# vladiant/CascadeClassifier

Measured on AMD Instinct MI355X. Metric: detection Mwindows/sec (1080p, haarcascade_frontalface) + achieved HBM GB/s, higher is better.
Workload: dtype i32+f32 (f64 stage sums)

## Files before the change

### cascadeclassifier_amd/_lib.py

```python
from __future__ import annotations

import ctypes as C
import os

_HERE = os.path.dirname(os.path.abspath(__file__))
LIB_PATH = os.environ.get("CCAMD_LIB") or os.path.join(_HERE, "lib", "libcascadeclassifier_amd.so")

CC_OK = 0
CC_ERR_INVALID_ARG = -1
CC_ERR_NO_DEVICE = -2
CC_ERR_HIP = -3
CC_ERR_IO = -4
CC_ERR_PARSE = -5
CC_ERR_UNSUPPORTED = -6
CC_ERR_BUFFER_TOO_SMALL = -7
CC_ERR_OUT_OF_RANGE = -8

CC_FEATURE_HAAR, CC_FEATURE_LBP, CC_FEATURE_HOG = 0, 1, 2
CC_PIX_GRAY8, CC_PIX_BGR8, CC_PIX_BGRA8, CC_PIX_RGB8, CC_PIX_RGBA8, CC_PIX_RGB8_PLANAR = 0, 1, 2, 3, 4, 5
CC_HAAR_BASIC, CC_HAAR_CORE, CC_HAAR_ALL = 0, 1, 2


class CascadeError(RuntimeError):

# ... 124 lines not shown
    "cc_detector_specialize": (_i, [_vp, _i]),
    "cc_detector_specialize_async": (_i, [_vp, _i]),
    "cc_detector_specialized_stages": (_i, [_vp]),
    "cc_cascade_compile_specialized": (_i, [_vp, _i, C.c_char_p, C.POINTER(C.c_size_t)]),
    "cc_detector_set_profiling": (_i, [_vp, _i]),
    "cc_detector_graph_active": (_i, [_vp]),
    "cc_detector_graph_captures": (C.c_int64, [_vp]),
    "cc_detector_get_timings": (_i, [_vp, C.POINTER(DetectorTimings), _i]),
    "cc_detector_candidate_capacity": (_i, [_vp]),
    "cc_integral_u8": (_i, [_i, _vp, _i, _i, _sz, _vp, _vp, _vp]),
    "cc_resize_linear_exact_u8": (_i, [_i, _vp, _i, _i, _sz, _vp, _i, _i, _sz]),
    "cc_debug_stream_dwords": (_i, [_i, _sz, _i, C.POINTER(C.c_uint32)]),
    "cc_debug_division_check": (_i, [_i, C.c_uint64, C.c_uint64, C.POINTER(C.c_uint64)]),
    "cc_debug_vnf_check": (_i, [_i, C.c_uint64, C.c_uint64, C.POINTER(C.c_uint64)]),
    "cc_debug_wave_int_tables": (_i, [_vp, _vp, _vp, _vp, _vp]),
    "cc_group_rectangles": (_i, [_vp, _i, _i, _d, _vp, _i, C.POINTER(_i)]),
    "cc_group_rectangles_device": (_i, [_i, _vp, _vp, _i, _i, _d, _vp, _i, _vp, C.POINTER(_i)]),
    "cc_group_rectangles_levels": (_i, [_vp, _vp, _vp, _i, _i, _d, _vp, _vp, _vp, _i, C.POINTER(_i)]),
    "cc_group_rectangles_device_levels": (_i, [_i, _vp, _vp, _vp, _vp, _i, _i, _d, _vp, _vp, _vp, _i, _vp, C.POINTER(_i)]),
    "cc_eval_create": (_i, [_i, _i, _i, _i, _i, _i, _pp]),
    "cc_eval_destroy": (None, [_vp]),
    "cc_eval_num_features": (_i, [_vp]),
    "cc_eval_max_cat_count": (_i, [_vp]),
    "cc_eval_feature_size": (_i, [_vp]),
    "cc_eval_feature_geometry": (_i, [_vp, _i, _vp, _vp, C.POINTER(_i)]),
    "cc_eval_set_image": (_i, [_vp, _vp, _sz, C.c_uint8, _i]),
    "cc_eval_set_images": (_i, [_vp, _vp, _i, _i, _vp]),
    "cc_eval_labels": (C.POINTER(C.c_float), [_vp]),
    "cc_eval_calc": (_i, [_vp, _i, _i, C.POINTER(C.c_float)]),
    "cc_eval_calc_list": (_i, [_vp, _vp, _i, _i, _vp]),
# ... 99 lines not shown
```

### cascadeclassifier_amd/csrc/cc_detect.hip

```cpp
#include <hip/hip_runtime.h>

#include <algorithm>

#include "cc_detector.h"

namespace ccamd {

#include "cc_eval_kernel.inc"

__global__ __launch_bounds__(256) void k_stream_dwords(const uint32_t* __restrict__ p, size_t n_words, uint32_t* __restrict__ out) {
  uint32_t acc = 0;
  for (size_t i = (size_t)blockIdx.x * blockDim.x + threadIdx.x; i < n_words; i += (size_t)gridDim.x * blockDim.x) acc += p[i];
  if (acc == 0x9e3779b9u) atomicAdd(out, acc);
  atomicAdd(out + 1 + (threadIdx.x & 15), acc);
}

__device__ __forceinline__ bool visited_by_scan(const unsigned long long* __restrict__ row_mask, int gx) {
  int run = 0;
  int pos = gx - 1;
  while (pos >= 0) {
    const int b = pos & 63;
    const unsigned long long w = row_mask[pos >> 6] << (63 - b);
    const int ones = min(__clzll((long long)~w), b + 1);
    run += ones;
// ... 115 lines not shown
  A.leaves = d->d_leaves.p;
  return A;
}

int eval_stamp_slots() { return STAMP_SLOTS; }

cc_status launch_eval(cc_detector* d, const Plan* P, int slot, int nchan, bool tilt, int sq_compact, bool debug, unsigned long long* stamps,
                      const EvalLaunch* launches, int n_launches, int nf, hipStream_t st) {
  const bool haar = d->m.feature_type == CC_FEATURE_HAAR;
  EvalArgs A = eval_args(d, P, slot, nchan, tilt, sq_compact, debug);
  A.stamps = stamps;
  for (int i = 0; i < n_launches; i++) {
    const EvalLaunch& L = launches[i];
    if (L.n_tiles == 0) continue;
    A.tiles = L.tiles;
    if (L.fn) {
      void* params[] = {&A};
      EvScope ev1(d, i == 1 ? EV_EVAL_STEP1 : -1, st);
      CC_HIP(hipModuleLaunchKernel(L.fn, (unsigned)L.n_tiles, (unsigned)nf, 1, EVAL_THREADS, 1, 1, (unsigned)L.lds, st, params, nullptr));
    } else if (haar)
      hipLaunchKernelGGL(k_eval_haar, dim3(L.n_tiles, nf), dim3(EVAL_THREADS), L.lds, st, A);
    else
      hipLaunchKernelGGL(k_eval_lbp, dim3(L.n_tiles, nf), dim3(EVAL_THREADS), L.lds, st, A);
    if (A.stamps) A.stamps += (size_t)L.n_tiles * (size_t)nf * STAMP_SLOTS;
  }
  return CC_OK;
}

void launch_filter_candidates(cc_detector* d, const Plan* P, int slot, hipStream_t st) {
  hipLaunchKernelGGL(k_filter_candidates, dim3(64), dim3(256), 0, st, d->d_cands[slot].p, d->d_counts[slot].p, d->cand_cap, P->front.d_sd.p,
// ... 64 lines not shown
```

### cascadeclassifier_amd/csrc/cc_detect_api.hip

```cpp
#include <algorithm>
#include <chrono>
#include <cstdlib>
#include <mutex>
#include <unordered_set>

#include "cc_detector.h"

namespace ccamd {

cc_status refuse_hog(const Cascade& m, const char* who) {
  if (m.feature_type == CC_FEATURE_HAAR || m.feature_type == CC_FEATURE_LBP) return CC_OK;
  return set_error(CC_ERR_UNSUPPORTED, "%s: %s cascades are not supported for detection (Haar and LBP only)", who,
                   m.feature_type == CC_FEATURE_HOG ? "HOG" : "unknown-type");
}

cc_status ensure_device(int device) {
  int n = 0;
  hipError_t e = hipGetDeviceCount(&n);
  if (e != hipSuccess || n <= 0)
    return set_error(CC_ERR_NO_DEVICE, "no usable HIP device (%s); this library has no CPU fallback",
                     e != hipSuccess ? hipGetErrorString(e) : "device count is 0");
  if (device < 0 || device >= n) return set_error(CC_ERR_INVALID_ARG, "device %d out of range (devices: %d)", device, n);
  CC_HIP(hipSetDevice(device));
  return CC_OK;
// ... 61 lines not shown
  sink->consume = [&cands](int, int, std::vector<CandOut>& c) { cands.insert(cands.end(), c.begin(), c.end()); };
  BatchOptions opt;
  opt.debug = debug;
  const cc_status st = run_batch(d, F, p, sink, opt);
  if (st == CC_OK) sort_candidates(cands);
  return st;
}

static cc_status spec_install(cc_detector* d, const std::vector<SpecCode>& codes, int k, int tmode) {
  retire_foreign(d);
  CC_HIP(hipStreamSynchronize(d->stream));
  SpecModule fresh[2];
  int n_fresh = 0;
  if (cc_status st = spec_load(d->m, codes, tmode, d->lds, fresh, &n_fresh); st != CC_OK) return st;
  d->unload_spec();
  for (int i = 0; i < n_fresh; i++) d->spec[i] = fresh[i];
  d->n_spec = n_fresh;
  d->spec_stages = k;
  return CC_OK;
}

static cc_status device_arch(int device, std::string& arch) {
  hipDeviceProp_t prop;
  CC_HIP(hipGetDeviceProperties(&prop, device));
  arch = prop.gcnArchName;
  arch = arch.substr(0, arch.find(':'));
  return CC_OK;
}

void spec_poll(cc_detector* d) {
  const int st = d->spec_bg_state.load(std::memory_order_acquire);
// ... 495 lines not shown
```

### cascadeclassifier_amd/csrc/cc_detect_internal.h

```cpp
#pragma once
#include <hip/hip_runtime.h>

#include <cstring>
#include <string>
#include <vector>

#include "cc_hip_util.h"
#include "cc_internal.h"

namespace ccamd {

#include "cc_eval_common.h"

__device__ __forceinline__ int find_segment(const int* __restrict__ first, int n, int idx) {
  int s = 0;
  while (s + 1 < n && first[s + 1] <= idx) s++;
  return s;
}

inline int align_up(int v, int a) { return (v + a - 1) / a * a; }

struct FrontLayout {
  int src_w = 0, src_h = 0;
  std::vector<ScaleDev> sd;
// ... 131 lines not shown

struct SpecCode {
  std::vector<char> code;
  int only_step = 0;
  int tile_y = TILE_Y;
};

cc_status spec_build(const Cascade& m, int n_stages, const std::string& arch, std::vector<SpecCode>& codes, int& k_out, int& tmode_out);

struct SpecModule {
  hipModule_t mod = nullptr;
  hipFunction_t fn = nullptr;
  size_t lds = 0;
  int tile_y = TILE_Y;
  int only_step = 0;
};

cc_status spec_load(const Cascade& m, const std::vector<SpecCode>& codes, int tmode, size_t base_lds, SpecModule out[2], int* n_out);

struct GroupGuard {
  const int* counts = nullptr;
  int cand_cap = 0;
  int* abort = nullptr;
};
constexpr int GROUP_WS_INTS = 7;
constexpr int GROUP_WS_INTS_SCORED = 10;
struct GroupScores {
  bool scored = false;
  const int32_t* levels = nullptr;
  int const_level = 0;
  const double* weights = nullptr;
// ... 18 lines not shown
```

### cascadeclassifier_amd/csrc/cc_detector.h

```cpp
#pragma once
#include <atomic>
#include <functional>
#include <future>
#include <map>
#include <memory>
#include <thread>

#include "cc_detect_internal.h"

namespace ccamd {

struct Plan {
  int w = 0, h = 0;
  cc_detect_params p{};
  std::vector<ScaleGeom> geom;
  FrontTables front;
  size_t mask_frame_words = 0;
  long long windows = 0, integral_elems = 0;
  int n_grid_rows = 0;
  struct TileList {
    int n = 0;
    DevBuf<int4> d;
  };
  std::map<std::pair<int, int>, TileList> tiles;
// ... 170 lines not shown
struct EvScope {
  cc_detector* d;
  int kind;
  OwnEvent a, b;
  hipStream_t st;
  EvScope(cc_detector* d_, int kind_, hipStream_t st_);
  ~EvScope();
};
void collect_events(cc_detector* d);

struct EvalLaunch {
  hipFunction_t fn;
  size_t lds;
  int n_tiles;
  const int4* tiles;
};
cc_status launch_eval(cc_detector* d, const Plan* P, int slot, int nchan, bool tilt, int sq_compact, bool debug, unsigned long long* stamps,
                      const EvalLaunch* launches, int n_launches, int nf, hipStream_t st);
int eval_stamp_slots();
void launch_filter_candidates(cc_detector* d, const Plan* P, int slot, hipStream_t st);
void launch_debug_visited(cc_detector* d, const Plan* P, int slot, hipStream_t st);
cc_status allow_large_lds(const cc_detector* d);

void configure_detector(cc_detector* d);
cc_status upload_cascade_tables(cc_detector* d);

cc_status build_plan(cc_detector* d, int w, int h, const cc_detect_params& p, Plan** out);
cc_status check_frame_args(const cc_detector* d, const FrameSet& F, const cc_detect_params* p, const char* who);
cc_status retire_pending(cc_detector* d);
void retire_foreign(cc_detector* d);
// ... 7 lines not shown
```

### cascadeclassifier_amd/csrc/cc_eval_common.h

```cpp
#ifndef CC_EVAL_COMMON_H
#define CC_EVAL_COMMON_H

constexpr int TILE_X = 64;
#ifndef CC_TILE_Y
#define CC_TILE_Y 8
#endif
#ifndef CC_EVAL_THREADS
#define CC_EVAL_THREADS 256
#endif
#ifndef CC_EVAL_MIN_WAVES_PER_EU
#define CC_EVAL_MIN_WAVES_PER_EU 5
#endif
constexpr int TILE_Y = CC_TILE_Y;
constexpr int EVAL_THREADS = CC_EVAL_THREADS;
constexpr int EVAL_WAVES = EVAL_THREADS / 64;
constexpr int WIN_PER_THREAD = TILE_Y / EVAL_WAVES;
constexpr int SPEC_PARTS = EVAL_WAVES >= 8 ? 8 : EVAL_WAVES >= 4 ? 4 : EVAL_WAVES >= 2 ? 2 : 1;

struct ScaleDev {
  int w, h;
  int pitch8, pitchI;
  long long img_ofs, int_ofs, mask_ofs, win_ofs, h_ofs;
  int ystep, nx, ny, nxw, nbands;
  float scale;
// ... 67 lines not shown
    rows = (tile_y - 1) * 2 + H0 + 1;
    rs16 = (cols + 3) / 4 * 4;
    if (rs16 % 16 == 0) rs16 += 4;
    row_stride = rs16 / 2;
  }
  __host__ __device__ int at(int r, int c) const { return r * rs16 + c; }
  __host__ __device__ int words() const { return rows * row_stride; }
};

constexpr int TILE_WINDOWS = TILE_X * TILE_Y;
constexpr int MAX_STAGES = 64;
constexpr int PART_DOUBLES = (EVAL_WAVES - 1) * 64;
constexpr int QUEUE_ROWS = TILE_WINDOWS / 32;
constexpr int VNF_PITCH = TILE_X + 32;
__host__ __device__ inline int tile_words_padded(int tile_words) { return (tile_words + 3) & ~3; }
__host__ __device__ inline size_t eval_lds_bytes(int tile_words, bool tilted, bool haar = true, int tile_y = TILE_Y) {
  return (size_t)tile_words_padded(tile_words) * 4 * (tilted ? 2 : 1) + PART_DOUBLES * 8 + (haar ? tile_y * VNF_PITCH * 4 : 0) +
         2 * (tile_y * TILE_X) * 2 + 3 * 32 * 4;
}

template <int CTRL, int ROW_MASK>
__device__ __forceinline__ double dpp_f64(double v) {
  const unsigned long long u = __double_as_longlong(v);
  const int lo = __builtin_amdgcn_update_dpp(0, (int)(unsigned)u, CTRL, ROW_MASK, 0xF, false);
  const int hi = __builtin_amdgcn_update_dpp(0, (int)(unsigned)(u >> 32), CTRL, ROW_MASK, 0xF, false);
  return __longlong_as_double(((unsigned long long)(unsigned)hi << 32) | (unsigned)lo);
}
__device__ __forceinline__ double readlane_f64(double v, int src) {
  const unsigned long long u = __double_as_longlong(v);
  const unsigned lo = __builtin_amdgcn_readlane((int)(unsigned)u, src);
  const unsigned hi = __builtin_amdgcn_readlane((int)(unsigned)(u >> 32), src);
  return __longlong_as_double(((unsigned long long)hi << 32) | lo);
}
// ... 15 lines not shown
```

### cascadeclassifier_amd/csrc/cc_eval_kernel.inc

```

#define CC_CONST __attribute__((address_space(4)))
template <class T>
__device__ __forceinline__ const T CC_CONST* as_const_table(const T* p) {
  return (const T CC_CONST*)p;
}
template <class T>
__device__ __forceinline__ T load_record(const T CC_CONST* p) {
  static_assert(sizeof(T) % 4 == 0, "table records are dword multiples");
  T out;
  const int CC_CONST* w = (const int CC_CONST*)p;
  int* o = reinterpret_cast<int*>(&out);
#pragma unroll
  for (unsigned i = 0; i < sizeof(T) / 4; i++) o[i] = w[i];
  return out;
}

constexpr int STAGE_ROWS = 12;
template <int STEP, class Geom>
__device__ __forceinline__ void stage_tile(int32_t* lds, const Geom& G, const int32_t* __restrict__ sum,
                                           const ScaleDev& S, int x0, int y0) {
  const int lane = threadIdx.x & 63, wave = __builtin_amdgcn_readfirstlane(threadIdx.x >> 6);
  const int quads = (G.cols + 3) >> 2;
  const bool right_edge = x0 + quads * 4 - 1 > S.w;
  for (int q0 = 0; q0 < quads; q0 += 64) {
// ... 262 lines not shown
#else
  static constexpr bool G16 = false;
#endif
  using Geom = typename cc_select<G16, TileGeom16, TileGeom<STEP>>::type;

  const EvalArgs& A;
  int32_t* const lds;
  const int4 T;
  const ScaleDev& S;
#ifdef CC_SPEC_W0
  static constexpr int W0 = CC_SPEC_W0, H0 = CC_SPEC_H0;
#else
  const int W0 = A.W0, H0 = A.H0;
#endif
  const Geom G{W0, H0};
  double* const s_part = reinterpret_cast<double*>(lds + tile_words_padded(G.words()) * ((HAAR && A.tilt_chan >= 0) ? 2 : 1));
  float* const s_vnf = reinterpret_cast<float*>(s_part + PART_DOUBLES);
  unsigned short* const s_q = reinterpret_cast<unsigned short*>(s_vnf + (HAAR ? TILE_Y * VNF_PITCH : 0));
  int* const s_cnt = reinterpret_cast<int*>(s_q + 2 * TILE_WINDOWS);
  const int frame = blockIdx.y;
  const int32_t* const sum = A.integ + ((size_t)frame * A.nchan + 0) * A.int_frame_elems + S.int_ofs;
  const int lane = threadIdx.x & 63, wave = __builtin_amdgcn_readfirstlane(threadIdx.x >> 6);
  const int half = lane >> 5, cls = lane & 31;
  const int gx0 = T.y * TILE_X, gy0 = T.z * TILE_Y;
  const int skew = (STEP * G.row_stride) & 31;
  const Node* const nodes = reinterpret_cast<const Node*>(STEP == 2 ? A.nodes2 : A.nodes1);
  const Stump CC_CONST* const stumps = as_const_table(reinterpret_cast<const Stump*>(G16 ? A.gstumps : STEP == 2 ? A.stumps2 : A.stumps1));
  const int CC_CONST* const stage_first = as_const_table(A.stage_first);
  const int CC_CONST* const stage_ntrees = as_const_table(A.stage_ntrees);
  const float CC_CONST* const stage_thr = as_const_table(A.stage_thr);
  const int CC_CONST* const group_first = as_const_table(A.group_first);
  const double CC_CONST* const wave_q = as_const_table(A.wave_q);
  const int CC_CONST* const wave_thr_q = as_const_table(A.wave_thr_q);
// ... 10 lines not shown
    if constexpr (G16)
      return GlobalReader{sum, (unsigned)((gy0 + (id >> 6)) * STEP) * (unsigned)S.pitchI + (unsigned)((gx0 + (id & 63)) * STEP), S.pitchI};
    else
      return LdsReader{lds + window_base(id)};
  }
  __device__ __forceinline__ void report(int id, int code, double last) const {
    const size_t o = (size_t)S.win_ofs + (size_t)(gy0 + (id >> 6)) * S.nx + (gx0 + (id & 63));
    A.dbg_codes[o] = code;
    if (A.dbg_sums) A.dbg_sums[o] = last;
  }
  __device__ __forceinline__ void emit_candidate(int id, double last_sum) const {
    const int slot = atomicAdd(A.cand_count, 1);
    if (slot < A.cand_cap) A.cands[slot] = CandRaw{frame, T.x, gx0 + (id & 63), gy0 + (id >> 6), last_sum};
  }
  __device__ __forceinline__ int win_class(int id) const { return ((id & 63) + skew * (id >> 6)) & 31; }
  __device__ __forceinline__ int vnf_slot(int id) const { return (id >> 6) * (TILE_X + skew) + (id & 63); }
  __device__ __forceinline__ void enqueue(bool pass, int id, int g) const {
    if (g >= A.dense_from) {
      const unsigned long long m = __ballot(pass);
      int first = 0;
      if (lane == 0 && m) first = atomicAdd(&s_cnt[(g % 3) * 32], __builtin_popcountll(m));
      first = __builtin_amdgcn_readfirstlane(first);
      if (pass) s_q[(g & 1) * TILE_WINDOWS + first + lane_rank(m)] = (unsigned short)id;
    } else if (pass) {
      const int c = win_class(id);
      const int row = atomicAdd(&s_cnt[(g % 3) * 32 + c], 1);
      s_q[(g & 1) * TILE_WINDOWS + row * 32 + c] = (unsigned short)id;
    }
  }
  __device__ __forceinline__ void deliver(bool pass, int id, double last_sum, bool last_group, int next_group) const {
    if (__builtin_expect(last_group, false)) {
      if (pass) {
        emit_candidate(id, last_sum);
        if (dbg) report(id, 1, last_sum);
      }
    } else
      enqueue(pass, id, next_group);
  }
  __device__ __forceinline__ bool never_visited(unsigned long long m) const {
    bool never = false;
    if (!dbg && A.early_skip) {
      const unsigned long long lower = (1ull << lane) - 1ull;
// ... 47 lines not shown
      if (lo == 0 || lo < nt) {
        Stump cur = load_record(stumps + first + lo);
        for (int j = lo; j < nt; j += step) {
          const Stump nxt = load_record(stumps + first + min(j + step, nt - 1));
          acc += stump_vote(rd, cur, vnf);
          cur = nxt;
        }
      }
    } else {
      for (int j = lo; j < nt; j += step) acc += stump_vote(rd, stumps + first + j, vnf);
    }
    return acc;
  }
  __device__ __forceinline__ WaveShare deal_windows(const QueueState& h) const {
    const unsigned short* q = s_q + (h.qg & 1) * TILE_WINDOWS;
    unsigned short* my_list = reinterpret_cast<unsigned short*>(s_part) + wave * 64;
    int numbered = 0;
    for (int r0 = 0; r0 < h.rows; r0 += 2) {
      const int row = r0 + half;
      const bool valid = row < h.my_rows;
      const int id = valid ? q[row * 32 + cls] : 0;
      const unsigned long long mask = __ballot(valid);
      const int number = numbered + lane_rank(mask);
      if (valid && number % EVAL_WAVES == wave) my_list[number / EVAL_WAVES] = (unsigned short)id;
      numbered += __builtin_popcountll(mask);
    }
    const int cnt = (numbered - wave + EVAL_WAVES - 1) / EVAL_WAVES;
    return WaveShare{cnt, lane < cnt ? my_list[lane] : 0, cnt >= 64 ? ~0ull : ((1ull << cnt) - 1ull)};
  }

  __device__ __forceinline__ void stage_phase(unsigned (&valsq_pre)[WIN_PER_THREAD]) const {
    unsigned sq_raw[WIN_PER_THREAD][4];
#pragma unroll
    for (int k = 0; k < WIN_PER_THREAD; k++) {
      sq_raw[k][0] = sq_raw[k][1] = sq_raw[k][2] = sq_raw[k][3] = 0;
      if (HAAR) {
// ... 171 lines not shown
        h.rows = wave_max_u32(h.my_rows);
        h.n = wave_sum_u32(h.my_rows) >> 1;
      }
      if (threadIdx.x < 32) s_cnt[((qg + 2) % 3) * 32 + threadIdx.x] = 0;
      if (st + 2 < STAMP_SLOTS - 1) stamp(st + 2);
      if (h.n == 0 || h.n < A.wave_below) break;
      const unsigned short* q = s_q + (qg & 1) * TILE_WINDOWS;
      const bool last_group = st_end >= A.nstages;
      const int groups = (h.rows + 1) >> 1;
      const bool may_split = A.split_stumps && st_end - st == 1;
      const int g_split = may_split ? groups - groups % EVAL_WAVES : groups;
      const int rem = groups - g_split;
      int ns = 1;
      if (rem > 0)
        while (ns * 2 * rem <= EVAL_WAVES) ns *= 2;
      const int g_end = ns == 1 ? groups : g_split;
      for (int g = wave; g < g_end; g += EVAL_WAVES) {
        const int row = g * 2 + half;
        const bool valid = row < h.my_rows;
        const int id = valid ? q[row * 32 + cls] : cls;
        const int32_t* b = lds + window_base(id);
        const float vnf = HAAR ? s_vnf[vnf_slot(id)] : 1.f;
        bool alive = valid;
        double acc = 0.;
        for (int s2 = st; s2 < st_end; s2++) {
          if (s2 > st && !__any(alive)) break;
          const double a = stage_sum(s2, id, b, vnf, alive);
          const bool pass = alive && !(a < (double)stage_thr[s2]);
          if (dbg && alive && !pass) report(id, -s2, a);
          if (alive) acc = a;
          alive = pass;
        }
        deliver(alive, id, acc, last_group, qg + 1);
      }
      if (ns > 1) split_stage(h, q, last_group, g_split, rem, ns);
    }
    return true;
  }
  __device__ __forceinline__ void split_stage(const QueueState& h, const unsigned short* q, bool last_group, int g_split, int rem, int ns) const {
    const int st = h.st;
    const int first = stage_first[st], nt = stage_ntrees[st];
    const int slice = wave % ns, grp = wave / ns;
    const int row = (g_split + grp) * 2 + half;
    const int i = grp * 64 + lane;
    const bool valid = row < h.my_rows;
    const int id = valid ? q[min(row, QUEUE_ROWS - 1) * 32 + cls] : cls;
    double acc = 0.;
    if (grp < rem) {
      [[maybe_unused]] const int32_t* b = lds + window_base(id);
      const float vnf = HAAR ? s_vnf[vnf_slot(id)] : 1.f;
#ifdef CC_SPEC_STAGES
      if (!TREES && st < CC_SPEC_STAGES)
        acc = spec_stage<STEP>(st, slice * (SPEC_PARTS / ns), (slice + 1) * (SPEC_PARTS / ns), b, vnf);
      else
#endif
        acc = table_sum(table_reader(id), first, nt, slice, ns, vnf);
      if (slice) s_part[(slice - 1) * (EVAL_THREADS / ns) + i] = acc;
    }
    __syncthreads();
    if (grp < rem && slice == 0) {
      for (int k = 1; k < ns; k++) acc += s_part[(k - 1) * (EVAL_THREADS / ns) + i];
      const bool pass = valid && !(acc < (double)stage_thr[st]);
      if (dbg && valid && !pass) report(id, -st, acc);
      deliver(pass, id, acc, last_group, h.qg + 1);
    }
  }

  template <class Acc>
  __device__ __forceinline__ Acc wave_stage(const Stump* wstumps, int s2, unsigned long long alive, int my_id) const {
    const int first = stage_first[s2], nt = stage_ntrees[s2];
    Acc tot = 0;
    for (int c = 0; c < nt; c += 64) {
      const int j = c + lane;
      const Stump rec = wstumps[first + min(j, nt - 1)];
      for (unsigned long long m = alive; m; m &= m - 1ull) {
        const int k = __builtin_ctzll(m);
// ... 179 lines not shown
```

### cascadeclassifier_amd/csrc/cc_pass.hip

```cpp
#include <algorithm>
#include <chrono>
#include <cstdlib>
#include <mutex>

#include "cc_detector.h"

namespace ccamd {

static bool same_params(const cc_detect_params& a, const cc_detect_params& b) {
  return a.scale_factor == b.scale_factor && a.min_w == b.min_w && a.min_h == b.min_h && a.max_w == b.max_w && a.max_h == b.max_h;
}

static std::vector<int4> plan_tile_list(const std::vector<ScaleGeom>& geom, int tile_y, int only_step) {
  std::vector<int4> tiles;
  for (size_t i = 0; i < geom.size(); i++) {
    const ScaleGeom& g = geom[i];
    if (only_step && g.ystep != only_step) continue;
    const int ntx = (g.nx + TILE_X - 1) / TILE_X, nty = (g.ny + tile_y - 1) / tile_y;
    for (int ty_ = 0; ty_ < nty; ty_++)
      for (int tx_ = 0; tx_ < ntx; tx_++) tiles.push_back(make_int4((int)i, tx_, ty_, 0));
  }
  const size_t n = tiles.size(), per = (n + 7) / 8;
  std::vector<int4> perm;
  perm.reserve(n);
// ... 98 lines not shown
      case EV_FILTER: d->tm.finalize_ms += ms; d->tm.finalize_launches++; break;
      case EV_GROUP: d->tm.group_ms += ms; d->tm.group_launches++; break;
    }
  }
  d->events.clear();
}

static cc_status pass_launches(cc_detector* d, Plan* P, bool create_lists, EvalLaunch out[2], int* n_out) {
  const bool run_spec = d->n_spec > 0 && d->m.max_nodes_per_tree <= 1;
  const int n = run_spec ? d->n_spec : 1;
  for (int i = 0; i < n; i++) {
    const SpecModule aot{nullptr, nullptr, d->lds, TILE_Y, 0};
    const SpecModule& M = run_spec ? d->spec[i] : aot;
    const Plan::TileList* tl = nullptr;
    if (cc_status st = plan_tiles(d, P, M.tile_y, M.only_step, create_lists, &tl); st != CC_OK) return st;
    out[i] = EvalLaunch{M.fn, M.lds, tl->n, tl->d.p};
  }
  *n_out = n;
  return CC_OK;
}

static cc_status ensure_spec_tiles(cc_detector* d, Plan* P) {
  EvalLaunch launches[2];
  int n = 0;
  return pass_launches(d, P, true, launches, &n);
}

static cc_status ensure_pass_workspace(cc_detector* d, const Plan* P, int slot, int nchan, bool tilt, bool debug) {
  const FrontLayout& FL = P->front.L;
  const size_t cap = (size_t)d->pass_capacity;
  CC_HIP(d->d_pyr.ensure(FL.pyr_frame_bytes * cap));
// ... 534 lines not shown
```

### cascadeclassifier_amd/csrc/cc_spec.hip

```cpp
#include <hip/hip_runtime.h>

#include <algorithm>
#include <array>
#include <cmath>
#include <cstdlib>
#include <cstring>
#include <map>
#include <mutex>

#include <dlfcn.h>
#include <sys/stat.h>
#include <unistd.h>

#include "cc_detect_internal.h"

namespace ccamd {

#include "build/cc_eval_kernel_src.h"

struct SpecStump {
  std::string loads;
  std::string decls;
  std::string compute;
  double base = 0.;
// ... 507 lines not shown
    api.code_size = reinterpret_cast<decltype(api.code_size)>(sym("hiprtcGetCodeSize"));
    api.code = reinterpret_cast<decltype(api.code)>(sym("hiprtcGetCode"));
    api.destroy = reinterpret_cast<decltype(api.destroy)>(sym("hiprtcDestroyProgram"));
    api.version = reinterpret_cast<decltype(api.version)>(sym("hiprtcVersion"));
  });
  return api;
}

static const char kSpecPrelude[] =
    "typedef signed char int8_t;\ntypedef unsigned char uint8_t;\ntypedef short int16_t;\ntypedef unsigned short uint16_t;\n"
    "typedef int int32_t;\ntypedef unsigned int uint32_t;\ntypedef long long int64_t;\ntypedef unsigned long long uint64_t;\n";

struct SpecModulePlan {
  int only_step, tile_y;
};
static std::vector<SpecModulePlan> spec_modules(const Cascade& m, int tmode) {
  auto valid = [&](int ty) { return ty >= EVAL_WAVES && ty <= 32 && ty % EVAL_WAVES == 0; };
  auto env_rows = [&](const char* name, int dflt) {
    const char* e = std::getenv(name);
    const int v = e ? std::atoi(e) : dflt;
    return valid(v) ? v : dflt;
  };
  if (m.has_tilted) return {{0, TILE_Y}};
  const bool lbp16 = m.feature_type == CC_FEATURE_LBP && tmode == TILE_16;
  const bool haar32 = tmode == TILE_32 && m.feature_type == CC_FEATURE_HAAR;
  const bool rows_given = std::getenv("CCAMD_SPEC_TILE_Y") != nullptr;
  const int all = env_rows("CCAMD_SPEC_TILE_Y", lbp16 ? 20 : TILE_Y);
  const bool two = (haar32 || std::getenv("CCAMD_SPEC_TWO_MODULES")) && !std::getenv("CCAMD_SPEC_ONE_MODULE");
  if (!two) return {{0, all}};
  return {{2, env_rows("CCAMD_SPEC_TILE_Y2", all)}, {1, env_rows("CCAMD_SPEC_TILE_Y1", (haar32 && !rows_given) ? 12 : all)}};
}

static cc_status compile_specialised(const std::string& src, const std::string& arch, int n_stages, bool lbp, int tmode, int tile_y, int only_step, int win_w, int win_h, std::vector<char>& code) {
  const bool tile16 = tmode == TILE_16;
  static std::mutex mu;
  static std::map<std::string, std::vector<char>> cache;
  const std::string o_arch = "--offload-arch=" + arch, o_k = "-DCC_SPEC_STAGES=" + std::to_string(n_stages);
  const std::string o_ty = "-DCC_TILE_Y=" + std::to_string(tile_y), o_th = "-DCC_EVAL_THREADS=" + std::to_string(EVAL_THREADS);
  const std::string o_w = "-DCC_EVAL_MIN_WAVES_PER_EU=" + std::to_string(tile16 ? (tile_y >= 20 ? 6 : 7) : CC_EVAL_MIN_WAVES_PER_EU);
  const std::string o_step = "-DCC_ONLY_STEP=" + std::to_string(only_step);
  const std::string o_w0 = "-DCC_SPEC_W0=" + std::to_string(win_w), o_h0 = "-DCC_SPEC_H0=" + std::to_string(win_h);
  std::vector<const char*> optv = {o_arch.c_str(), "-O3", "-std=c++17", "-ffp-contract=off", "-fno-fast-math", o_k.c_str(), o_ty.c_str(), o_th.c_str(), o_w.c_str(), o_w0.c_str(), o_h0.c_str()};
  if (only_step) optv.push_back(o_step.c_str());
  if (lbp) optv.push_back("-DCC_SPEC_LBP");
  if (tile16) optv.push_back("-DCC_SPEC_TILE16");
  const char* const* opts = optv.data();
  const int n_opts = (int)optv.size();
  std::string key;
  {
    int major = 0, minor = 0;
    const HipRtcApi& rtc = hiprtc_api();
    if (rtc.version) (void)rtc.version(&major, &minor);
    key += "hiprtc " + std::to_string(major) + "." + std::to_string(minor) + " ";
  }
  for (int i = 0; i < n_opts; i++) key += std::string(opts[i]) + " ";
  key += "#" + src;
  {
    std::lock_guard<std::mutex> lk(mu);
    auto it = cache.find(key);
    if (it != cache.end()) {
// ... 108 lines not shown
  src += "namespace ccamd {\n";
  src += kEvalKernelSrc;
  src += "\n}  // namespace ccamd\n";
  const std::string marker = "//@@CC_SPEC_FUNCTIONS@@";
  const size_t pos = src.find(marker);
  if (pos == std::string::npos) return set_error(CC_ERR_HIP, "cc_detector_specialize: kernel source has no specialisation marker");
  const int tmode = tile16_eligible(m, k) ? TILE_16 : TILE_32;
  src.replace(pos, marker.size(), spec_stage_source(m, k, tmode));
  k_out = k;
  tmode_out = tmode;
  codes.clear();
  for (const SpecModulePlan& mp : spec_modules(m, tmode)) {
    SpecCode c;
    c.only_step = mp.only_step;
    c.tile_y = mp.tile_y;
    const cc_status st = compile_specialised(src, arch, k, m.feature_type == CC_FEATURE_LBP, tmode, mp.tile_y, mp.only_step, m.win_w, m.win_h, c.code);
    if (st != CC_OK) return st;
    codes.push_back(std::move(c));
  }
  return CC_OK;
}

cc_status spec_load(const Cascade& m, const std::vector<SpecCode>& codes, int tmode, size_t base_lds, SpecModule out[2], int* n_out) {
  if (codes.empty() || codes.size() > 2) return set_error(CC_ERR_HIP, "cc_detector_specialize: %zu modules", codes.size());
  const bool haar_k = m.feature_type == CC_FEATURE_HAAR;
  int n = 0;
  auto fail = [&](SpecModule& x) {
    (void)hipGetLastError();
    if (x.mod) (void)hipModuleUnload(x.mod);
    for (int i = 0; i < n; i++) (void)hipModuleUnload(out[i].mod);
  };
  for (const SpecCode& c : codes) {
    SpecModule x;
    x.tile_y = c.tile_y;
    x.only_step = c.only_step;
    const char* entry = c.only_step == 1 ? "k_eval_spec_step1" : c.only_step == 2 ? "k_eval_spec_step2" : "k_eval_spec";
    if (hipModuleLoadData(&x.mod, c.code.data()) != hipSuccess || hipModuleGetFunction(&x.fn, x.mod, entry) != hipSuccess) {
      fail(x);
      return set_error(CC_ERR_HIP, "cc_detector_specialize: the compiled module does not load or has no entry point");
    }
    const int ty = c.tile_y, step = c.only_step;
    x.lds = base_lds;
    if (tmode == TILE_32) {
      const TileGeom<1> G1(m.win_w, m.win_h, ty);
      const TileGeom<2> G2(m.win_w, m.win_h, ty);
      const int words = step == 1 ? G1.words() : step == 2 ? G2.words() : std::max(G1.words(), G2.words());
      x.lds = eval_lds_bytes(words, m.has_tilted, haar_k, ty);
    } else if (tmode == TILE_16) {
      const TileGeom<1> G1(m.win_w, m.win_h, ty);
      const TileGeom16 G2(m.win_w, m.win_h, ty);
      x.lds = eval_lds_bytes(std::max(G1.words(), G2.words()), false, haar_k, ty);
    }
    if (x.lds > 64 * 1024) {
      const hipError_t e = hipFuncSetAttribute(reinterpret_cast<const void*>(x.fn), hipFuncAttributeMaxDynamicSharedMemorySize, (int)x.lds);
      if (e != hipSuccess) {
        fail(x);
        return set_error(CC_ERR_UNSUPPORTED, "cc_detector_specialize: %zu bytes of LDS per tile cannot be requested for a run-time module (%s)",
                         x.lds, hipGetErrorString(e));
      }
    }
    if (std::getenv("CCAMD_TRACE_HOST")) {
      int nb = 0;
// ... 1 lines not shown
      std::fprintf(stderr, "[ccamd host] specialised kernel: tile mode %d, tiles of step %d (0 = all), %d window rows, %zu bytes of LDS per block, %d resident blocks per CU\n",
                   tmode, c.only_step, ty, x.lds, nb);
    }
    out[n++] = x;
  }
  if (n == 2 && out[0].only_step == 1) std::swap(out[0], out[1]);
  *n_out = n;
  return CC_OK;
}

}

using namespace ccamd;

extern "C" {

cc_status cc_cascade_compile_specialized(const cc_cascade* c, int n_stages, const char* arch, size_t* code_bytes) {
  if (!c || !arch || !code_bytes) return set_error(CC_ERR_INVALID_ARG, "cc_cascade_compile_specialized: null argument");
  if (cc_status hs = refuse_hog(c->m, "cc_cascade_compile_specialized"); hs != CC_OK) return hs;
  std::vector<SpecCode> code;
  int k = 0;
  int tmode = 0;
  const cc_status st = spec_build(c->m, std::max(1, n_stages), arch, code, k, tmode);
  if (st != CC_OK) return st;
  *code_bytes = 0;
  for (const SpecCode& m : code) *code_bytes += m.code.size();
  return CC_OK;
}

}
// ... 1 lines not shown
```

### include/cascadeclassifier_amd.h

```cpp
#ifndef CASCADECLASSIFIER_AMD_H_
#define CASCADECLASSIFIER_AMD_H_

#include <stddef.h>
#include <stdint.h>

#ifdef __cplusplus
extern "C" {
#endif

#if defined(__GNUC__)
#define CC_API __attribute__((visibility("default")))
#else
#define CC_API
#endif

typedef int cc_status;
enum {
  CC_OK = 0,
  CC_ERR_INVALID_ARG = -1,
  CC_ERR_NO_DEVICE = -2,
  CC_ERR_HIP = -3,
  CC_ERR_IO = -4,
  CC_ERR_PARSE = -5,
  CC_ERR_UNSUPPORTED = -6,
// ... 145 lines not shown
CC_API int cc_detector_graph_active(const cc_detector* d);
CC_API int64_t cc_detector_graph_captures(const cc_detector* d);

CC_API cc_status cc_integral_u8(int device, const uint8_t* img, int width, int height, size_t row_stride, int32_t* sum,
                                int32_t* sqsum, int32_t* tilted);
CC_API cc_status cc_resize_linear_exact_u8(int device, const uint8_t* src, int sw, int sh, size_t sstride, uint8_t* dst,
                                           int dw, int dh, size_t dstride);
CC_API cc_status cc_warp_perspective_u8(int device, const uint8_t* src, int sw, int sh, size_t sstride, uint8_t* dst, int dw,
                                        int dh, size_t dstride, const double* quad);
CC_API cc_status cc_to_gray_u8(int device, const uint8_t* src, int pixel_format, int width, int height, size_t row_stride,
                               uint8_t* dst, size_t dst_stride);
CC_API cc_status cc_debug_stream_dwords(int device, size_t n_bytes, int repeats, uint32_t* checksum);
CC_API cc_status cc_debug_division_check(int device, uint64_t n_pairs, uint64_t seed, uint64_t* mismatches);
CC_API cc_status cc_debug_vnf_check(int device, uint64_t n_values, uint64_t seed, uint64_t* mismatches);
CC_API cc_status cc_debug_wave_int_tables(const cc_cascade* c, double* q, int32_t* thr_q, int32_t* left_q, int32_t* right_q);
CC_API cc_status cc_group_rectangles(const cc_rect* rects, int n, int group_threshold, double eps, cc_rect* out, int cap,
                                     int* n_out);
CC_API cc_status cc_group_rectangles_device(int device, const cc_rect* rects, const int32_t* offsets, int n_frames,
                                            int group_threshold, double eps, cc_rect* out, int cap, int32_t* out_offsets,
                                            int* n_total);
CC_API cc_status cc_group_rectangles_levels(const cc_rect* rects, const int32_t* levels, const double* weights, int n,
                                            int group_threshold, double eps, cc_rect* out, int32_t* out_levels,
                                            double* out_weights, int cap, int* n_out);
CC_API cc_status cc_group_rectangles_device_levels(int device, const cc_rect* rects, const int32_t* levels,
                                                   const double* weights, const int32_t* offsets, int n_frames,
                                                   int group_threshold, double eps, cc_rect* out, int32_t* out_levels,
                                                   double* out_weights, int cap, int32_t* out_offsets, int* n_total);

typedef struct cc_evaluator cc_evaluator;
enum { CC_HAAR_BASIC = 0, CC_HAAR_CORE = 1, CC_HAAR_ALL = 2 };
// ... 188 lines not shown
```

Measured before the change: 19300.

## Add lean LDS layout for step-1 Haar specialised kernel and taller tiles

```diff
diff --git a/cascadeclassifier_amd/_lib.py b/cascadeclassifier_amd/_lib.py
--- a/cascadeclassifier_amd/_lib.py
+++ b/cascadeclassifier_amd/_lib.py
@@ -162,6 +162,7 @@
     "cc_debug_division_check": (_i, [_i, C.c_uint64, C.c_uint64, C.POINTER(C.c_uint64)]),
     "cc_debug_vnf_check": (_i, [_i, C.c_uint64, C.c_uint64, C.POINTER(C.c_uint64)]),
     "cc_debug_wave_int_tables": (_i, [_vp, _vp, _vp, _vp, _vp]),
+    "cc_debug_spec_step1_plan": (_i, [_vp, _i, _i, _vp, _vp, _vp, _vp]),
     "cc_group_rectangles": (_i, [_vp, _i, _i, _d, _vp, _i, C.POINTER(_i)]),
     "cc_group_rectangles_device": (_i, [_i, _vp, _vp, _i, _i, _d, _vp, _i, _vp, C.POINTER(_i)]),
     "cc_group_rectangles_levels": (_i, [_vp, _vp, _vp, _i, _i, _d, _vp, _vp, _vp, _i, C.POINTER(_i)]),
diff --git a/cascadeclassifier_amd/csrc/cc_detect.hip b/cascadeclassifier_amd/csrc/cc_detect.hip
--- a/cascadeclassifier_amd/csrc/cc_detect.hip
+++ b/cascadeclassifier_amd/csrc/cc_detect.hip
@@ -153,6 +153,7 @@
     const EvalLaunch& L = launches[i];
     if (L.n_tiles == 0) continue;
     A.tiles = L.tiles;
+    A.wave_below = L.wave_below >= 0 ? L.wave_below : d->wave_below;
     if (L.fn) {
       void* params[] = {&A};
       EvScope ev1(d, i == 1 ? EV_EVAL_STEP1 : -1, st);
diff --git a/cascadeclassifier_amd/csrc/cc_detect_api.hip b/cascadeclassifier_amd/csrc/cc_detect_api.hip
--- a/cascadeclassifier_amd/csrc/cc_detect_api.hip
+++ b/cascadeclassifier_amd/csrc/cc_detect_api.hip
@@ -99,7 +99,10 @@
   int n_fresh = 0;
   if (cc_status st = spec_load(d->m, codes, tmode, d->lds, fresh, &n_fresh); st != CC_OK) return st;
   d->unload_spec();
-  for (int i = 0; i < n_fresh; i++) d->spec[i] = fresh[i];
+  for (int i = 0; i < n_fresh; i++) {
+    d->spec[i] = fresh[i];
+    d->spec[i].wave_below = spec_wave_below(d->wave_below, fresh[i].only_step, fresh[i].tile_y);
+  }
   d->n_spec = n_fresh;
   d->spec_stages = k;
   return CC_OK;
diff --git a/cascadeclassifier_amd/csrc/cc_detect_internal.h b/cascadeclassifier_amd/csrc/cc_detect_internal.h
--- a/cascadeclassifier_amd/csrc/cc_detect_internal.h
+++ b/cascadeclassifier_amd/csrc/cc_detect_internal.h
@@ -169,7 +169,10 @@
   size_t lds = 0;
   int tile_y = TILE_Y;
   int only_step = 0;
-};
+  int wave_below = -1;
+};
+
+int spec_wave_below(int detector_value, int only_step, int tile_y);
 
 cc_status spec_load(const Cascade& m, const std::vector<SpecCode>& codes, int tmode, size_t base_lds, SpecModule out[2], int* n_out);
 
diff --git a/cascadeclassifier_amd/csrc/cc_detector.h b/cascadeclassifier_amd/csrc/cc_detector.h
--- a/cascadeclassifier_amd/csrc/cc_detector.h
+++ b/cascadeclassifier_amd/csrc/cc_detector.h
@@ -208,6 +208,7 @@
   size_t lds;
   int n_tiles;
   const int4* tiles;
+  int wave_below = -1;
 };
 cc_status launch_eval(cc_detector* d, const Plan* P, int slot, int nchan, bool tilt, int sq_compact, bool debug, unsigned long long* stamps,
                       const EvalLaunch* launches, int n_launches, int nf, hipStream_t st);
diff --git a/cascadeclassifier_amd/csrc/cc_eval_common.h b/cascadeclassifier_amd/csrc/cc_eval_common.h
--- a/cascadeclassifier_amd/csrc/cc_eval_common.h
+++ b/cascadeclassifier_amd/csrc/cc_eval_common.h
@@ -105,9 +105,17 @@
 constexpr int QUEUE_ROWS = TILE_WINDOWS / 32;
 constexpr int VNF_PITCH = TILE_X + 32;
 __host__ __device__ inline int tile_words_padded(int tile_words) { return (tile_words + 3) & ~3; }
-__host__ __device__ inline size_t eval_lds_bytes(int tile_words, bool tilted, bool haar = true, int tile_y = TILE_Y) {
+__host__ __device__ inline size_t eval_lds_bytes(int tile_words, bool tilted, bool haar = true, int tile_y = TILE_Y, bool lean = false) {
+  if (lean) return (size_t)tile_words_padded(tile_words) * 4 + tile_y * TILE_X * 4 + 2 * (tile_y * TILE_X) * 2 + 3 * 32 * 4;
   return (size_t)tile_words_padded(tile_words) * 4 * (tilted ? 2 : 1) + PART_DOUBLES * 8 + (haar ? tile_y * VNF_PITCH * 4 : 0) +
          2 * (tile_y * TILE_X) * 2 + 3 * 32 * 4;
+}
+__host__ __device__ inline int lean_split_gap_bytes(int tile_y, int rows) { return 2 * (tile_y * TILE_X) * 2 - 2 * rows * 32 * 2; }
+__host__ __device__ inline int split_part_bytes(int ns) { return (ns - 1) * (EVAL_THREADS / ns) * 8; }
+constexpr int CU_LDS_BYTES = 160 * 1024;
+__host__ __device__ inline int lds_blocks_per_cu(size_t lds_bytes) {
+  const int n = (int)((size_t)CU_LDS_BYTES / (lds_bytes ? lds_bytes : 1)), cap = 32 / EVAL_WAVES;
+  return n > cap ? cap : n;
 }
 
 template <int CTRL, int ROW_MASK>
diff --git a/cascadeclassifier_amd/csrc/cc_eval_kernel.inc b/cascadeclassifier_amd/csrc/cc_eval_kernel.inc
--- a/cascadeclassifier_amd/csrc/cc_eval_kernel.inc
+++ b/cascadeclassifier_amd/csrc/cc_eval_kernel.inc
@@ -300,9 +300,14 @@
   const int W0 = A.W0, H0 = A.H0;
 #endif
   const Geom G{W0, H0};
-  double* const s_part = reinterpret_cast<double*>(lds + tile_words_padded(G.words()) * ((HAAR && A.tilt_chan >= 0) ? 2 : 1));
-  float* const s_vnf = reinterpret_cast<float*>(s_part + PART_DOUBLES);
-  unsigned short* const s_q = reinterpret_cast<unsigned short*>(s_vnf + (HAAR ? TILE_Y * VNF_PITCH : 0));
+#ifdef CC_LEAN_LDS
+  static constexpr bool kLean = HAAR && !TREES && STEP == 1;
+#else
+  static constexpr bool kLean = false;
+#endif
+  double* const s_part = kLean ? nullptr : reinterpret_cast<double*>(lds + tile_words_padded(G.words()) * ((HAAR && A.tilt_chan >= 0) ? 2 : 1));
+  float* const s_vnf = kLean ? reinterpret_cast<float*>(lds + tile_words_padded(G.words())) : reinterpret_cast<float*>(s_part + PART_DOUBLES);
+  unsigned short* const s_q = reinterpret_cast<unsigned short*>(s_vnf + (HAAR ? TILE_Y * (kLean ? TILE_X : VNF_PITCH) : 0));
   int* const s_cnt = reinterpret_cast<int*>(s_q + 2 * TILE_WINDOWS);
   const int frame = blockIdx.y;
   const int32_t* const sum = A.integ + ((size_t)frame * A.nchan + 0) * A.int_frame_elems + S.int_ofs;
@@ -343,18 +348,54 @@
     if (slot < A.cand_cap) A.cands[slot] = CandRaw{frame, T.x, gx0 + (id & 63), gy0 + (id >> 6), last_sum};
   }
   __device__ __forceinline__ int win_class(int id) const { return ((id & 63) + skew * (id >> 6)) & 31; }
-  __device__ __forceinline__ int vnf_slot(int id) const { return (id >> 6) * (TILE_X + skew) + (id & 63); }
+  __device__ __forceinline__ int vnf_slot(int id) const {
+    if constexpr (kLean)
+      return (id & ~63) | (((id & 63) + skew * (id >> 6)) & 63);
+    else
+      return (id >> 6) * (TILE_X + skew) + (id & 63);
+  }
+  __device__ __forceinline__ int q_index(int g, int row, int c) const {
+    if constexpr (kLean)
+      return (g & 1) ? (2 * QUEUE_ROWS - 1 - row) * 32 + c : row * 32 + c;
+    else
+      return (g & 1) * TILE_WINDOWS + row * 32 + c;
+  }
+  __device__ __forceinline__ int queued(const unsigned short* q, int g, int row, int c) const {
+    if constexpr (kLean)
+      return s_q[q_index(g, row, c)];
+    else
+      return q[row * 32 + c];
+  }
+  __device__ __forceinline__ double* split_parts(int rows) const {
+    if constexpr (kLean)
+      return reinterpret_cast<double*>(s_q + rows * 32);
+    else
+      return s_part;
+  }
+  __device__ __forceinline__ unsigned short* wave_lists(int qg) const {
+    if constexpr (kLean)
+      return s_q + ((qg & 1) ? 0 : 2 * TILE_WINDOWS - EVAL_WAVES * 64);
+    else
+      return reinterpret_cast<unsigned short*>(s_part);
+  }
   __device__ __forceinline__ void enqueue(bool pass, int id, int g) const {
     if (g >= A.dense_from) {
       const unsigned long long m = __ballot(pass);
       int first = 0;
       if (lane == 0 && m) first = atomicAdd(&s_cnt[(g % 3) * 32], __builtin_popcountll(m));
       first = __builtin_amdgcn_readfirstlane(first);
-      if (pass) s_q[(g & 1) * TILE_WINDOWS + first + lane_rank(m)] = (unsigned short)id;
+      if constexpr (kLean) {
+        const int i = first + lane_rank(m);
+        if (pass) s_q[q_index(g, i >> 5, i & 31)] = (unsigned short)id;
+      } else if (pass)
+        s_q[(g & 1) * TILE_WINDOWS + first + lane_rank(m)] = (unsigned short)id;
     } else if (pass) {
       const int c = win_class(id);
       const int row = atomicAdd(&s_cnt[(g % 3) * 32 + c], 1);
-      s_q[(g & 1) * TILE_WINDOWS + row * 32 + c] = (unsigned short)id;
+      if constexpr (kLean)
+        s_q[q_index(g, row, c)] = (unsigned short)id;
+      else
+        s_q[(g & 1) * TILE_WINDOWS + row * 32 + c] = (unsigned short)id;
     }
   }
   __device__ __forceinline__ void deliver(bool pass, int id, double last_sum, bool last_group, int next_group) const {
@@ -432,12 +473,12 @@
   }
   __device__ __forceinline__ WaveShare deal_windows(const QueueState& h) const {
     const unsigned short* q = s_q + (h.qg & 1) * TILE_WINDOWS;
-    unsigned short* my_list = reinterpret_cast<unsigned short*>(s_part) + wave * 64;
+    unsigned short* my_list = wave_lists(h.qg) + wave * 64;
     int numbered = 0;
     for (int r0 = 0; r0 < h.rows; r0 += 2) {
       const int row = r0 + half;
       const bool valid = row < h.my_rows;
-      const int id = valid ? q[row * 32 + cls] : 0;
+      const int id = valid ? queued(q, h.qg, row, cls) : 0;
       const unsigned long long mask = __ballot(valid);
       const int number = numbered + lane_rank(mask);
       if (valid && number % EVAL_WAVES == wave) my_list[number / EVAL_WAVES] = (unsigned short)id;
@@ -639,11 +680,13 @@
       int ns = 1;
       if (rem > 0)
         while (ns * 2 * rem <= EVAL_WAVES) ns *= 2;
+      if constexpr (kLean)
+        while (ns > 1 && split_part_bytes(ns) > lean_split_gap_bytes(TILE_Y, h.rows)) ns >>= 1;
       const int g_end = ns == 1 ? groups : g_split;
       for (int g = wave; g < g_end; g += EVAL_WAVES) {
         const int row = g * 2 + half;
         const bool valid = row < h.my_rows;
-        const int id = valid ? q[row * 32 + cls] : cls;
+        const int id = valid ? queued(q, qg, row, cls) : cls;
         const int32_t* b = lds + window_base(id);
         const float vnf = HAAR ? s_vnf[vnf_slot(id)] : 1.f;
         bool alive = valid;
@@ -669,7 +712,7 @@
     const int row = (g_split + grp) * 2 + half;
     const int i = grp * 64 + lane;
     const bool valid = row < h.my_rows;
-    const int id = valid ? q[min(row, QUEUE_ROWS - 1) * 32 + cls] : cls;
+    const int id = valid ? queued(q, h.qg, min(row, QUEUE_ROWS - 1), cls) : cls;
     double acc = 0.;
     if (grp < rem) {
       [[maybe_unused]] const int32_t* b = lds + window_base(id);
@@ -680,11 +723,11 @@
       else
 #endif
         acc = table_sum(table_reader(id), first, nt, slice, ns, vnf);
-      if (slice) s_part[(slice - 1) * (EVAL_THREADS / ns) + i] = acc;
+      if (slice) split_parts(h.rows)[(slice - 1) * (EVAL_THREADS / ns) + i] = acc;
     }
     __syncthreads();
     if (grp < rem && slice == 0) {
-      for (int k = 1; k < ns; k++) acc += s_part[(k - 1) * (EVAL_THREADS / ns) + i];
+      for (int k = 1; k < ns; k++) acc += split_parts(h.rows)[(k - 1) * (EVAL_THREADS / ns) + i];
       const bool pass = valid && !(acc < (double)stage_thr[st]);
       if (dbg && valid && !pass) report(id, -st, acc);
       deliver(pass, id, acc, last_group, h.qg + 1);
diff --git a/cascadeclassifier_amd/csrc/cc_pass.hip b/cascadeclassifier_amd/csrc/cc_pass.hip
--- a/cascadeclassifier_amd/csrc/cc_pass.hip
+++ b/cascadeclassifier_amd/csrc/cc_pass.hip
@@ -136,7 +136,7 @@
     const SpecModule& M = run_spec ? d->spec[i] : aot;
     const Plan::TileList* tl = nullptr;
     if (cc_status st = plan_tiles(d, P, M.tile_y, M.only_step, create_lists, &tl); st != CC_OK) return st;
-    out[i] = EvalLaunch{M.fn, M.lds, tl->n, tl->d.p};
+    out[i] = EvalLaunch{M.fn, M.lds, tl->n, tl->d.p, M.wave_below};
   }
   *n_out = n;
   return CC_OK;
diff --git a/cascadeclassifier_amd/csrc/cc_spec.hip b/cascadeclassifier_amd/csrc/cc_spec.hip
--- a/cascadeclassifier_amd/csrc/cc_spec.hip
+++ b/cascadeclassifier_amd/csrc/cc_spec.hip
@@ -545,6 +545,27 @@
 struct SpecModulePlan {
   int only_step, tile_y;
 };
+static bool spec_lean_lds(const Cascade& m, int tmode, int only_step) {
+  return only_step == 1 && tmode == TILE_32 && m.feature_type == CC_FEATURE_HAAR && !m.has_tilted;
+}
+static size_t spec_step1_lds(const Cascade& m, int tile_y) {
+  return eval_lds_bytes(TileGeom<1>(m.win_w, m.win_h, tile_y).words(), false, true, tile_y, true);
+}
+constexpr int kSpecStep1Rows = 20;
+constexpr int kSpecStep1MinBlocks = 4;
+static int spec_step1_rows(const Cascade& m, int want) {
+  int ty = want;
+  while (ty - EVAL_WAVES >= TILE_Y && lds_blocks_per_cu(spec_step1_lds(m, ty)) < kSpecStep1MinBlocks) ty -= EVAL_WAVES;
+  return ty;
+}
+constexpr int kStep1WaveBelow = 32;
+int spec_wave_below(int detector_value, int only_step, int tile_y) {
+  if (only_step != 1 || detector_value <= 0) return -1;
+  if (const char* e = std::getenv("CCAMD_WAVE_BELOW1")) return std::max(0, std::min(64, std::atoi(e)));
+  if (std::getenv("CCAMD_WAVE_BELOW") || tile_y < 12) return -1;
+  return std::max(detector_value, kStep1WaveBelow);
+}
+
 static std::vector<SpecModulePlan> spec_modules(const Cascade& m, int tmode) {
   auto valid = [&](int ty) { return ty >= EVAL_WAVES && ty <= 32 && ty % EVAL_WAVES == 0; };
   auto env_rows = [&](const char* name, int dflt) {
@@ -559,22 +580,29 @@
   const int all = env_rows("CCAMD_SPEC_TILE_Y", lbp16 ? 20 : TILE_Y);
   const bool two = (haar32 || std::getenv("CCAMD_SPEC_TWO_MODULES")) && !std::getenv("CCAMD_SPEC_ONE_MODULE");
   if (!two) return {{0, all}};
-  return {{2, env_rows("CCAMD_SPEC_TILE_Y2", all)}, {1, env_rows("CCAMD_SPEC_TILE_Y1", (haar32 && !rows_given) ? 12 : all)}};
-}
-
-static cc_status compile_specialised(const std::string& src, const std::string& arch, int n_stages, bool lbp, int tmode, int tile_y, int only_step, int win_w, int win_h, std::vector<char>& code) {
+  return {{2, env_rows("CCAMD_SPEC_TILE_Y2", all)}, {1, env_rows("CCAMD_SPEC_TILE_Y1", (haar32 && !rows_given) ? spec_step1_rows(m, kSpecStep1Rows) : all)}};
+}
+
+static cc_status compile_specialised(const std::string& src, const std::string& arch, int n_stages, bool lbp, int tmode, int tile_y, int only_step, int win_w, int win_h,
+                                     int lean_blocks, std::vector<char>& code) {
   const bool tile16 = tmode == TILE_16;
   static std::mutex mu;
   static std::map<std::string, std::vector<char>> cache;
   const std::string o_arch = "--offload-arch=" + arch, o_k = "-DCC_SPEC_STAGES=" + std::to_string(n_stages);
   const std::string o_ty = "-DCC_TILE_Y=" + std::to_string(tile_y), o_th = "-DCC_EVAL_THREADS=" + std::to_string(EVAL_THREADS);
-  const std::string o_w = "-DCC_EVAL_MIN_WAVES_PER_EU=" + std::to_string(tile16 ? (tile_y >= 20 ? 6 : 7) : CC_EVAL_MIN_WAVES_PER_EU);
+  int min_waves = tile16 ? (tile_y >= 20 ? 6 : 7) : CC_EVAL_MIN_WAVES_PER_EU;
+  if (lean_blocks > 0) {
+    min_waves = std::max(1, std::min(8, lean_blocks * EVAL_WAVES / 4));
+    if (const char* e = std::getenv("CCAMD_SPEC_WAVES1")) min_waves = std::max(1, std::min(8, std::atoi(e)));
+  }
+  const std::string o_w = "-DCC_EVAL_MIN_WAVES_PER_EU=" + std::to_string(min_waves);
   const std::string o_step = "-DCC_ONLY_STEP=" + std::to_string(only_step);
   const std::string o_w0 = "-DCC_SPEC_W0=" + std::to_string(win_w), o_h0 = "-DCC_SPEC_H0=" + std::to_string(win_h);
   std::vector<const char*> optv = {o_arch.c_str(), "-O3", "-std=c++17", "-ffp-contract=off", "-fno-fast-math", o_k.c_str(), o_ty.c_str(), o_th.c_str(), o_w.c_str(), o_w0.c_str(), o_h0.c_str()};
   if (only_step) optv.push_back(o_step.c_str());
   if (lbp) optv.push_back("-DCC_SPEC_LBP");
   if (tile16) optv.push_back("-DCC_SPEC_TILE16");
+  if (lean_blocks > 0) optv.push_back("-DCC_LEAN_LDS");
   const char* const* opts = optv.data();
   const int n_opts = (int)optv.size();
   std::string key;
@@ -713,7 +741,8 @@
     SpecCode c;
     c.only_step = mp.only_step;
     c.tile_y = mp.tile_y;
-    const cc_status st = compile_specialised(src, arch, k, m.feature_type == CC_FEATURE_LBP, tmode, mp.tile_y, mp.only_step, m.win_w, m.win_h, c.code);
+    const int lean_blocks = spec_lean_lds(m, tmode, mp.only_step) ? std::max(1, lds_blocks_per_cu(spec_step1_lds(m, mp.tile_y))) : 0;
+    const cc_status st = compile_specialised(src, arch, k, m.feature_type == CC_FEATURE_LBP, tmode, mp.tile_y, mp.only_step, m.win_w, m.win_h, lean_blocks, c.code);
     if (st != CC_OK) return st;
     codes.push_back(std::move(c));
   }
@@ -744,7 +773,7 @@
       const TileGeom<1> G1(m.win_w, m.win_h, ty);
       const TileGeom<2> G2(m.win_w, m.win_h, ty);
       const int words = step == 1 ? G1.words() : step == 2 ? G2.words() : std::max(G1.words(), G2.words());
-      x.lds = eval_lds_bytes(words, m.has_tilted, haar_k, ty);
+      x.lds = spec_lean_lds(m, tmode, step) ? spec_step1_lds(m, ty) : eval_lds_bytes(words, m.has_tilted, haar_k, ty);
     } else if (tmode == TILE_16) {
       const TileGeom<1> G1(m.win_w, m.win_h, ty);
       const TileGeom16 G2(m.win_w, m.win_h, ty);
@@ -776,6 +805,25 @@
 using namespace ccamd;
 
 extern "C" {
+
+cc_status cc_debug_spec_step1_plan(const cc_cascade* c, int rows_wanted, int wave_below_detector, int* rows, size_t* lds_bytes, int* blocks_per_cu,
+                                   int* wave_below) {
+  if (!c) return set_error(CC_ERR_INVALID_ARG, "cc_debug_spec_step1_plan: null cascade");
+  if (cc_status hs = refuse_hog(c->m, "cc_debug_spec_step1_plan"); hs != CC_OK) return hs;
+  if (c->m.max_nodes_per_tree > 1 || !spec_lean_lds(c->m, TILE_32, 1))
+    return set_error(CC_ERR_UNSUPPORTED, "cc_debug_spec_step1_plan: upright Haar stump cascades only");
+  const int ty = rows_wanted > 0 ? rows_wanted : spec_step1_rows(c->m, kSpecStep1Rows);
+  if (ty < EVAL_WAVES || ty > 32 || ty % EVAL_WAVES) return set_error(CC_ERR_INVALID_ARG, "cc_debug_spec_step1_plan: %d window rows per tile", ty);
+  const size_t lds = spec_step1_lds(c->m, ty);
+  if (rows) *rows = ty;
+  if (lds_bytes) *lds_bytes = lds;
+  if (blocks_per_cu) *blocks_per_cu = lds_blocks_per_cu(lds);
+  if (wave_below) {
+    const int w = spec_wave_below(wave_below_detector, 1, ty);
+    *wave_below = w >= 0 ? w : wave_below_detector;
+  }
+  return CC_OK;
+}
 
 cc_status cc_cascade_compile_specialized(const cc_cascade* c, int n_stages, const char* arch, size_t* code_bytes) {
   if (!c || !arch || !code_bytes) return set_error(CC_ERR_INVALID_ARG, "cc_cascade_compile_specialized: null argument");
diff --git a/include/cascadeclassifier_amd.h b/include/cascadeclassifier_amd.h
--- a/include/cascadeclassifier_amd.h
+++ b/include/cascadeclassifier_amd.h
@@ -183,6 +183,8 @@
 CC_API cc_status cc_debug_division_check(int device, uint64_t n_pairs, uint64_t seed, uint64_t* mismatches);
 CC_API cc_status cc_debug_vnf_check(int device, uint64_t n_values, uint64_t seed, uint64_t* mismatches);
 CC_API cc_status cc_debug_wave_int_tables(const cc_cascade* c, double* q, int32_t* thr_q, int32_t* left_q, int32_t* right_q);
+CC_API cc_status cc_debug_spec_step1_plan(const cc_cascade* c, int rows_wanted, int wave_below_detector, int* rows, size_t* lds_bytes,
+                                          int* blocks_per_cu, int* wave_below);
 CC_API cc_status cc_group_rectangles(const cc_rect* rects, int n, int group_threshold, double eps, cc_rect* out, int cap,
                                      int* n_out);
 CC_API cc_status cc_group_rectangles_device(int device, const cc_rect* rects, const int32_t* offsets, int n_frames,
```

Result: faster. 20180, median of 6 (+4.5%).
